# arnauqb/GradABM-JUNE

Hardware: AMD Instinct MI355X
Metric: simulation steps/sec (higher is better)
Workload: dtype f32

## Files before the change

### gradabm-june_amd/csrc/gj_tiled.h

```cpp
#pragma once
#include <hip/hip_runtime.h>
#include <stdint.h>

#include "../../include/gradjune_hip.h"
#include "gj_device.h"

namespace gj {

constexpr int kTileThreads = 1024;
constexpr int kTileWaves = kTileThreads / kWave;
constexpr int kMaxSliceAgents = 19840;
constexpr int kUnroll = 8;
#ifndef GJ_UNROLL_NARROW
#define GJ_UNROLL_NARROW 16
#endif
constexpr int kUnrollNarrow = GJ_UNROLL_NARROW;
#ifndef GJ_VENUE_UNROLL
#define GJ_VENUE_UNROLL 2
#endif
constexpr int kVenueUnroll = GJ_VENUE_UNROLL;
#ifndef GJ_VENUE_UNROLL_C
#define GJ_VENUE_UNROLL_C GJ_VENUE_UNROLL
#endif
constexpr int kVenueUnrollC = GJ_VENUE_UNROLL_C;
// ... 135 lines not shown
  b = (lane >= ((d1.z >> 24) & 0xFF)) ? d1.x : b;
  b = (lane >= (d1.w & 0xFF)) ? d1.y : b;
  return b + lane;
}
__device__ __noinline__ int chunk_slot_walk(const TSetA& T, int row, int i, int j) {
  while (i >= T.tile_sptr[row + j + 1]) ++j;
  return T.tile_jpos[row + j] + (i - T.tile_sptr[row + j]);
}

template <bool WIDE, int U>
__device__ __forceinline__ int batch_desc_load(const TSetA& T, int c_base, int n_chunks, int c0, int lane) {
  constexpr int W = WIDE ? 8 : 4;
  static_assert(U * W <= kWave, "a batch's descriptors must fit one wave-wide load");
  const int32_t* desc = reinterpret_cast<const int32_t*>(T.chunk_desc);
  const int u_l = min(lane / W, U - 1), k_l = lane % W;
  return at32(desc, (c_base + min(c0 + u_l, n_chunks - 1)) * W + k_l);
}

template <bool WIDE, int U>
__device__ __forceinline__ void batch_slots(const TSetA& T, const int word, int row, int seg0, int seg1, int c0,
                                            int lane, int (&slot)[U]) {
  constexpr int W = WIDE ? 8 : 4;
  const int k_l = lane % W;
  const bool flag = WIDE ? (k_l == 7 && (word & 0x100)) : (k_l == 2 && (word >> 16));
  const bool any_multi = __builtin_amdgcn_ballot_w64(flag) != 0ull;
#define GJ_DW(u, k) __builtin_amdgcn_readlane(word, (u) * W + (k))
  if (!any_multi) {
#pragma unroll
    for (int u = 0; u < U; ++u) {
      if (!WIDE) {
        slot[u] = chunk_slot_fast(make_int4(GJ_DW(u, 0), GJ_DW(u, 1), GJ_DW(u, 2), 0), lane);
      } else {
        slot[u] = chunk_slot_wide(make_int4(GJ_DW(u, 0), GJ_DW(u, 1), GJ_DW(u, 2), GJ_DW(u, 3)),
                                  make_int4(GJ_DW(u, 4), GJ_DW(u, 5), GJ_DW(u, 6), GJ_DW(u, 7)), lane);
      }
    }
  } else if (T.multi_slots) {
    int ms[U];
    bool mu[U];
#pragma unroll
    for (int u = 0; u < U; ++u) {
      const int w = WIDE ? GJ_DW(u, 7) : GJ_DW(u, 2);
      mu[u] = WIDE ? ((w & 0x100) != 0) : ((w >> 16) != 0);
      const int j0 = WIDE ? (int)((unsigned)w >> 9) : GJ_DW(u, 3);
      ms[u] = at32(T.multi_slots, (mu[u] ? j0 : 0) * kWave + lane);
    }
#pragma unroll
    for (int u = 0; u < U; ++u) {
      int f;
      if (!WIDE) {
        f = chunk_slot_fast(make_int4(GJ_DW(u, 0), GJ_DW(u, 1), GJ_DW(u, 2), 0), lane);
      } else {
        f = chunk_slot_wide(make_int4(GJ_DW(u, 0), GJ_DW(u, 1), GJ_DW(u, 2), GJ_DW(u, 3)),
                            make_int4(GJ_DW(u, 4), GJ_DW(u, 5), GJ_DW(u, 6), GJ_DW(u, 7)), lane);
      }
      slot[u] = mu[u] ? ms[u] : f;
    }
  } else {
#pragma unroll
    for (int u = 0; u < U; ++u) {
      const int i = min(seg0 + (c0 + u) * kWave + lane, seg1 - 1);
      if (!WIDE) {
        const int4 d = make_int4(GJ_DW(u, 0), GJ_DW(u, 1), GJ_DW(u, 2), GJ_DW(u, 3));
        slot[u] = (d.z >> 16) ? chunk_slot_slow(T, d, row, i, lane) : chunk_slot_fast(d, lane);
      } else {
        const int4 d0 = make_int4(GJ_DW(u, 0), GJ_DW(u, 1), GJ_DW(u, 2), GJ_DW(u, 3));
        const int4 d1 = make_int4(GJ_DW(u, 4), GJ_DW(u, 5), GJ_DW(u, 6), GJ_DW(u, 7));
        slot[u] = (d1.w & 0x100) ? chunk_slot_walk(T, row, i, (int)((unsigned)d1.w >> 9))
                                 : chunk_slot_wide(d0, d1, lane);
      }
    }
  }
#undef GJ_DW
}

#ifndef GJ_SCATTER_PIPELINE
#define GJ_SCATTER_PIPELINE 1
#endif
template <bool WIDE, int kU, bool NT = false>
__device__ __forceinline__ void scatter_batches(const TSetA& T, const float* lds_x, int s, int wave, int lane) {
  const int row = s * T.J;
  const int seg0 = T.tile_sptr[row], seg1 = T.tile_sptr[row + T.J];
  const int c_base = T.chunk_ptr[s];
  const int n_chunks = T.chunk_ptr[s + 1] - c_base;
  constexpr int kStride = kTileWaves * kU;
  auto stage1 = [&](int c, int& word, int (&la)[kU]) {
    const int cc = min(c, n_chunks - 1);
    word = batch_desc_load<WIDE, kU>(T, c_base, n_chunks, cc, lane);
#pragma unroll
    for (int u = 0; u < kU; ++u) la[u] = at32(T.a_la, min(seg0 + (cc + u) * kWave + lane, seg1 - 1));
  };
  auto stage2 = [&](int c, int word, const int (&la)[kU]) {
    int slot[kU];
    batch_slots<WIDE, kU>(T, word, row, seg0, seg1, c, lane, slot);
#ifdef GJ_DIAG_EXTRA_VALU
#pragma unroll
    for (int u = 0; u < kU; ++u)
#pragma unroll
      for (int r = 0; r < GJ_DIAG_EXTRA_VALU; ++r) asm volatile("v_add_u32 %0, %0, 0" : "+v"(slot[u]));
#endif
#pragma unroll
    for (int u = 0; u < kU; ++u) {
      const int i = seg0 + (c + u) * kWave + lane;
      if ((c + u < n_chunks) && (i < seg1)) {
        if (NT) put32nt(T.val, slot[u], lds_x[la[u]]); else put32(T.val, slot[u], lds_x[la[u]]);
      }
    }
  };
  int c0 = wave * kU;
  if (c0 >= n_chunks) return;
  int laA[kU], wordA;
#if GJ_SCATTER_PIPELINE
  int laB[kU], wordB;
  stage1(c0, wordA, laA);
  while (true) {
    const int c1 = c0 + kStride;
    stage1(c1, wordB, laB);
    stage2(c0, wordA, laA);
    if (c1 >= n_chunks) break;
    const int c2 = c1 + kStride;
    stage1(c2, wordA, laA);
    stage2(c1, wordB, laB);
    if (c2 >= n_chunks) break;
    c0 = c2;
  }
#else
  for (; c0 < n_chunks; c0 += kStride) {
    stage1(c0, wordA, laA);
    stage2(c0, wordA, laA);
  }
#endif
}

constexpr int kLongSegmentChunks = 384;
#ifndef GJ_NT_TILE_EDGES
#define GJ_NT_TILE_EDGES 1024
#endif
constexpr int kNtTileEdges = GJ_NT_TILE_EDGES;
template <bool WIDE>
__device__ __forceinline__ void scatter_set(const TSetA& T, const float* lds_x, int s, int wave, int lane) {
  const int n_chunks = T.chunk_ptr[s + 1] - T.chunk_ptr[s];
  if (!WIDE && kUnrollNarrow != kUnroll && n_chunks >= kLongSegmentChunks && n_chunks * kWave >= kNtTileEdges * T.J) {
    scatter_batches<WIDE, WIDE ? kUnroll : kUnrollNarrow, true>(T, lds_x, s, wave, lane);
  } else if (!WIDE && kUnrollNarrow != kUnroll && n_chunks >= kLongSegmentChunks) {
    scatter_batches<WIDE, WIDE ? kUnroll : kUnrollNarrow>(T, lds_x, s, wave, lane);
  } else {
    scatter_batches<WIDE, kUnroll>(T, lds_x, s, wave, lane);
  }
}

#ifndef GJ_UNROLL_D_NARROW
#define GJ_UNROLL_D_NARROW 8
#endif
#ifndef GJ_GATHER_PIPELINE
#define GJ_GATHER_PIPELINE 1
#endif
template <bool WIDE>
__device__ __forceinline__ void gather_set(const TSetA& T, fx_t* lds_acc, uint32_t* lds_flags, int flag_words, int s,
                                           int wave, int lane) {
  const int row = s * T.J;
  const int seg0 = T.tile_sptr[row], seg1 = T.tile_sptr[row + T.J];
  const int c_base = T.chunk_ptr[s];
  const int n_chunks = T.chunk_ptr[s + 1] - c_base;
  constexpr int kU = WIDE ? kUnroll : GJ_UNROLL_D_NARROW;
  constexpr int kStride = kTileWaves * kU;
  auto stage1 = [&](int c, int& word, int (&la)[kU]) {
    const int cc = min(c, n_chunks - 1);
    word = batch_desc_load<WIDE, kU>(T, c_base, n_chunks, cc, lane);
#pragma unroll
    for (int u = 0; u < kU; ++u) la[u] = at32(T.a_la, min(seg0 + (cc + u) * kWave + lane, seg1 - 1));
  };
  auto values = [&](int c, int word, float (&v)[kU]) {
    int slot[kU];
    batch_slots<WIDE, kU>(T, word, row, seg0, seg1, c, lane, slot);
#pragma unroll
    for (int u = 0; u < kU; ++u) {
      const int i = seg0 + (c + u) * kWave + lane;
      const bool ok = (c + u < n_chunks) && (i < seg1);
      v[u] = at32nt(T.val, ok ? slot[u] : 0);
    }
  };
  auto add = [&](int c, const int (&la)[kU], const float (&v)[kU]) {
    constexpr uint32_t kLimit = 0x48800000u;
    static_assert(kFxAgent == 32, "kLimit is the pattern of 2^(50 - kFxAgent)");
    float x[kU];
    uint32_t m = 0u;
#pragma unroll
    for (int u = 0; u < kU; ++u) {
      const int i = seg0 + (c + u) * kWave + lane;
      const bool edge = (c + u < n_chunks) && (i < seg1);
      x[u] = edge ? v[u] : 0.0f;
      m = max(m, __float_as_uint(x[u]) & 0x7FFFFFFFu);
    }
#ifdef GJ_DIAG_EXTRA_VALU
#pragma unroll
    for (int u = 0; u < kU; ++u)
#pragma unroll
      for (int r = 0; r < GJ_DIAG_EXTRA_VALU; ++r) asm volatile("v_add_f32 %0, %0, 0" : "+v"(x[u]));
#endif
    if (__builtin_expect(m <= kLimit, 1)) {
#pragma unroll
      for (int u = 0; u < kU; ++u) atomicAdd(&lds_acc[la[u]], to_fx<kFxAgent>(x[u]));
    } else {
#pragma unroll
      for (int u = 0; u < kU; ++u) {
        if ((__float_as_uint(x[u]) & 0x7FFFFFFFu) <= kLimit) {
          atomicAdd(&lds_acc[la[u]], to_fx<kFxAgent>(x[u]));
        } else {
          fx_flag(lds_flags, flag_words, la[u], x[u]);
        }
      }
    }
  };
  int c0 = wave * kU;
  if (c0 >= n_chunks) return;
  int laA[kU], wordA;
  float v[kU];
#if GJ_GATHER_PIPELINE
  int laB[kU], wordB;
  stage1(c0, wordA, laA);
  while (true) {
    const int c1 = c0 + kStride;
    values(c0, wordA, v);
    stage1(c1, wordB, laB);
    add(c0, laA, v);
    if (c1 >= n_chunks) break;
    const int c2 = c1 + kStride;
    values(c1, wordB, v);
    stage1(c2, wordA, laA);
    add(c1, laB, v);
    if (c2 >= n_chunks) break;
    c0 = c2;
  }
#else
  for (; c0 < n_chunks; c0 += kStride) {
    stage1(c0, wordA, laA);
    values(c0, wordA, v);
    add(c0, laA, v);
  }
#endif
}

template <int kU>
__device__ __forceinline__ void scatter_explicit(const TSetA& T, const float* lds_x, int s, int wave, int lane) {
  const int row = s * T.J;
  const int seg0 = T.tile_sptr[row], seg1 = T.tile_sptr[row + T.J];
  const int n_chunks = T.chunk_ptr[s + 1] - T.chunk_ptr[s];
  const int32_t* slots = reinterpret_cast<const int32_t*>(T.chunk_desc);
  for (int c0 = wave * kU; c0 < n_chunks; c0 += kTileWaves * kU) {
    int la[kU], sl[kU];
#pragma unroll
    for (int u = 0; u < kU; ++u) {
      const int i = min(seg0 + (c0 + u) * kWave + lane, seg1 - 1);
      la[u] = at32(T.a_la, i);
      sl[u] = at32(slots, i);
    }
#pragma unroll
    for (int u = 0; u < kU; ++u) {
      const int i = seg0 + (c0 + u) * kWave + lane;
      if ((c0 + u < n_chunks) && (i < seg1)) put32(T.val, sl[u], lds_x[la[u]]);
    }
  }
}

template <int kU>
__device__ __forceinline__ void gather_explicit(const TSetA& T, fx_t* lds_acc, uint32_t* lds_flags, int flag_words, int s,
                                                int wave, int lane) {
  const int row = s * T.J;
  const int seg0 = T.tile_sptr[row], seg1 = T.tile_sptr[row + T.J];
  const int n_chunks = T.chunk_ptr[s + 1] - T.chunk_ptr[s];
  const int32_t* slots = reinterpret_cast<const int32_t*>(T.chunk_desc);
  constexpr uint32_t kLimit = 0x48800000u;
  for (int c0 = wave * kU; c0 < n_chunks; c0 += kTileWaves * kU) {
    int la[kU], sl[kU];
#pragma unroll
    for (int u = 0; u < kU; ++u) {
      const int i = min(seg0 + (c0 + u) * kWave + lane, seg1 - 1);
      la[u] = at32(T.a_la, i);
      sl[u] = at32(slots, i);
    }
    float x[kU];
#pragma unroll
    for (int u = 0; u < kU; ++u) x[u] = at32(T.val, sl[u]);
    uint32_t m = 0u;
#pragma unroll
    for (int u = 0; u < kU; ++u) {
      const int i = seg0 + (c0 + u) * kWave + lane;
      x[u] = ((c0 + u < n_chunks) && (i < seg1)) ? x[u] : 0.0f;
      m = max(m, __float_as_uint(x[u]) & 0x7FFFFFFFu);
    }
    if (__builtin_expect(m <= kLimit, 1)) {
#pragma unroll
      for (int u = 0; u < kU; ++u) atomicAdd(&lds_acc[la[u]], to_fx<kFxAgent>(x[u]));
    } else {
#pragma unroll
      for (int u = 0; u < kU; ++u) {
        if ((__float_as_uint(x[u]) & 0x7FFFFFFFu) <= kLimit) {
          atomicAdd(&lds_acc[la[u]], to_fx<kFxAgent>(x[u]));
        } else {
          fx_flag(lds_flags, flag_words, la[u], x[u]);
        }
      }
    }
  }
}

#ifndef GJ_SCATTER_WAVES_PER_SIMD
#define GJ_SCATTER_WAVES_PER_SIMD 4
#endif
__global__ __launch_bounds__(kTileThreads, GJ_SCATTER_WAVES_PER_SIMD) void k_tile_scatter(const TileAArgs A) {
  extern __shared__ __align__(16) float lds_x[];
  const int tid = threadIdx.x;
  const int wave = __builtin_amdgcn_readfirstlane(tid / kWave), lane = tid % kWave;
  const int s = blockIdx.x;
  const int64_t base = (int64_t)s * A.slice_agents;
  const int n_local = (int)min((int64_t)A.slice_agents, A.n_agents - base);
  const bool two_sources = A.qtrans != A.trans;
  for (int pass = 0; pass < 2; ++pass) {
    if (pass == 1 && !two_sources) break;
    bool any = false;
    for (int t = 0; t < A.n_sets; ++t)
      if (A.sets[t].active && !A.sets[t].presum && (!two_sources || A.sets[t].raw == pass)) any = true;
    if (!any) continue;
    if (pass == 1) __syncthreads();
    load_slice(lds_x, pass == 0 ? A.qtrans : A.trans, base, n_local, tid);
    __syncthreads();
    for (int t = 0; t < A.n_sets; ++t) {
      const TSetA& T = A.sets[t];
      if (!T.active || T.presum || (two_sources && T.raw != pass)) continue;
      if (T.wide == 2) {
        scatter_explicit<kUnroll>(T, lds_x, s, wave, lane);
      } else if (T.wide) {
        scatter_set<true>(T, lds_x, s, wave, lane);
      } else {
        scatter_set<false>(T, lds_x, s, wave, lane);
      }
    }
  }
}

struct TSetB {
  const int32_t* blk_v0;
  const int32_t* blk_e0;
  const uint16_t* e_lv;
  const uint8_t* e_cls;
  float* val;
  const float* v_pc;
  float* cum;
  int32_t stride;
  int32_t nk;
  float beta[GJ_MAX_NETS_PER_SET];
  int32_t table[GJ_MAX_NETS_PER_SET];
  int32_t age75[GJ_MAX_NETS_PER_SET];
  int32_t leisure;
  int32_t direct;
  uint32_t term_limit;
  int32_t _pad_b;
  const uint16_t* pv_blk;
  const int32_t* blk_r0;
  const float* x;
  int64_t n_x;
};

struct TileBArgs {
  TSetB sets[GJ_MAX_SETS];
  const int32_t* work;
  const float* tables;
  int32_t day_type;
  int32_t mode;
  int32_t transpose;
  int32_t _pad;
};

__device__ __noinline__ void venue_group_slow(fx_t* sums, uint32_t* vflags, int words, uint32_t limit, int base_k, int l0,
                                              int l1, int l2, int l3, int l4, int l5, int l6, int l7, float x0, float x1,
                                              float x2, float x3, float x4, float x5, float x6, float x7) {
  const int lv[8] = {l0, l1, l2, l3, l4, l5, l6, l7};
  const float x[8] = {x0, x1, x2, x3, x4, x5, x6, x7};
#pragma unroll
  for (int q = 0; q < 8; ++q) {
    if (lv[q] == 0xFFFF) continue;
    if ((__float_as_uint(x[q]) & 0x7FFFFFFFu) <= limit) {
      atomicAdd(&sums[base_k + lv[q]], to_fx<kFxVenue>(x[q]));
    } else {
      fx_flag(vflags, words, base_k + lv[q], x[q]);
    }
  }
}

struct Slots8 {
  uint32_t w[4];
  __device__ __forceinline__ int lv(int q) const { return (w[q >> 1] >> ((q & 1) * 16)) & 0xFFFF; }
};

#ifdef GJ_DIAG_STAMPS
constexpr int kDiagVenueSlots = 8192;
__device__ unsigned long long gj_diag_venue[3 * kDiagVenueSlots];
struct VenueStamp {
  unsigned long long t0;
  __device__ VenueStamp() : t0(__builtin_amdgcn_s_memrealtime()) {}
  __device__ ~VenueStamp() {
    if (threadIdx.x == 0 && blockIdx.x < kDiagVenueSlots) {
      gj_diag_venue[3 * blockIdx.x] = t0;
      gj_diag_venue[3 * blockIdx.x + 1] = __builtin_amdgcn_s_memrealtime();
      gj_diag_venue[3 * blockIdx.x + 2] = __builtin_amdgcn_s_getreg((31 << 11) | 20) & 0xF;
    }
  }
};
#endif

#ifndef GJ_VENUE_WAVES_PER_SIMD
#define GJ_VENUE_WAVES_PER_SIMD 4
#endif
__global__ __launch_bounds__(kTileThreads, GJ_VENUE_WAVES_PER_SIMD) void k_tile_venues(const TileBArgs B) {
  extern __shared__ __align__(16) float lds_s[];
#ifdef GJ_DIAG_STAMPS
  VenueStamp gj_stamp;
#endif
  const int tid = threadIdx.x;
  const int set = B.work[2 * blockIdx.x], j = B.work[2 * blockIdx.x + 1];
  const TSetB& T = B.sets[set];
  const int nk = T.nk;
  if (nk == 0) return;
  const int v0 = T.blk_v0[j], nv = T.blk_v0[j + 1] - v0;
  const int g0 = T.blk_e0[j] >> 3, g1 = T.blk_e0[j + 1] >> 3;
  fx_t* sums = reinterpret_cast<fx_t*>(lds_s);
  float* cumf = lds_s;
  float* tabs = lds_s + 2 * ((size_t)nk * nv + 64);
  uint32_t* vflags = reinterpret_cast<uint32_t*>(tabs + (T.leisure ? 2 * nk * 200 : 0));
  const int vwords = (nk * nv + 64 + 31) / 32;
  if (T.leisure) {
    for (int i = tid; i < nk * 200; i += kTileThreads) {
      const int k = i / 200, c = i % 200;
      const float l = B.tables[(int64_t)T.table[k] * GJ_TABLE_SIZE + B.day_type * 200 + c];
      const float lw = T.age75[k] ? l * (((c % 100) > 75) ? 1.0f : 0.0f) : l;
      tabs[i] = B.transpose ? lw : l;
      tabs[nk * 200 + i] = B.transpose ? l : lw;
    }
  }
  const uint4* lv8 = reinterpret_cast<const uint4*>(T.e_lv);
  const uint2* cls8 = reinterpret_cast<const uint2*>(T.e_cls);
  float4* val4 = reinterpret_cast<float4*>(T.val);
  if (B.mode != 2) {
    for (int i = tid; i < nk * nv + 64; i += kTileThreads) sums[i] = 0;
    for (int i = tid; i < 2 * vwords; i += kTileThreads) vflags[i] = 0u;
    __syncthreads();
    const int dummy = nk * nv + (tid & 63);
#if defined(GJ_DIAG_FLOAT_RUNS)
    auto run_sums = [&](const int (&lv)[8], const float (&x)[8], int base_k) {
      float s8 = x[0];
#pragma unroll
      for (int q = 0; q < 8; ++q) {
        const bool last = (q == 7) || (lv[q + (q < 7)] != lv[q]);
        const bool take = last && lv[q] != 0xFFFF;
        fx_add<kFxVenue>(sums, vflags, vwords, take ? base_k + lv[q] : dummy, take ? s8 : 0.0f);
// ... 544 lines not shown
        for (int c = 0; c < K; ++c) x[j][c] = tab[idx[j][c] * stride];
    } else {
#pragma unroll
      for (int j = 0; j < 4; ++j)
#pragma unroll
        for (int c = 0; c < K; ++c) x[j][c] = 0.0f;
#pragma unroll
      for (int k = 0; k < GJ_MAX_NETS_PER_SET; ++k) {
        if (k >= nk) break;
        float w[4];
#pragma unroll
        for (int j = 0; j < 4; ++j) w[j] = wtab[k * 200 + ((b.cls[u] >> (8 * j)) & 0xFF)];
#pragma unroll
        for (int j = 0; j < 4; ++j)
#pragma unroll
          for (int c = 0; c < K; ++c) x[j][c] += w[j] * tab[idx[j][c] * stride + k];
      }
    }
#pragma unroll
    for (int j = 0; j < 4; ++j) {
      float sj = 0.0f;
#pragma unroll
      for (int c = 0; c < K; ++c) sj += ok[j][c] ? x[j][c] : 0.0f;
      acc[u][j] += sj;
    }
  }
}

__device__ __forceinline__ void direct_stage(const TileDArgs& D, const TDirect& T, float* wtab, float* tab, int v0,
                                             int nv, int tid) {
  if (T.leisure && v0 == 0) {
    for (int i = tid; i < T.nk * 200; i += kTileThreads) {
      const int k = i / 200, c = i % 200;
      const float l = D.tables[(int64_t)T.table[k] * GJ_TABLE_SIZE + D.day_type * 200 + c];
      const float lw = T.age75[k] ? l * (((c % 100) > 75) ? 1.0f : 0.0f) : l;
      wtab[i] = D.transpose ? l : lw;
    }
  }
#ifndef GJ_DIAG_NO_DIRECT_TABLE
  const float* src = T.cum + (int64_t)v0 * T.stride;
  const int n = nv * T.stride;
  const int lane = tid % kWave, wave = __builtin_amdgcn_readfirstlane(tid / kWave);
#if GJ_DMA_WIDE
  const bool aligned = ((reinterpret_cast<uintptr_t>(src) | reinterpret_cast<uintptr_t>(tab)) & 15u) == 0;
  const int n_wide = aligned ? (n / (4 * kWave)) * (4 * kWave) : 0;
  for (int p = wave; (p + 1) * 4 * kWave <= n_wide; p += kTileWaves)
    __builtin_amdgcn_global_load_lds(src + p * 4 * kWave + 4 * lane, tab + p * 4 * kWave, 16, 0, 0);
  for (int p = wave; n_wide + p * kWave < n; p += kTileWaves)
    __builtin_amdgcn_global_load_lds(src + min(n_wide + p * kWave + lane, n - 1), tab + n_wide + p * kWave, 4, 0, 0);
#else
  for (int p = wave; p * kWave < n; p += kTileWaves)
    __builtin_amdgcn_global_load_lds(src + min(p * kWave + lane, n - 1), tab + p * kWave, 4, 0, 0);
#endif
#endif
}

__device__ __forceinline__ void publish_staged() {
  asm volatile("s_waitcnt vmcnt(0)" ::: "memory");
  __syncthreads();
}

__device__ __forceinline__ bool direct_next(const TileDArgs& D, int& t, int& v0, int& plane) {
  const TDirect& T = D.direct[t];
  if (plane + 1 < T.planes) {
    ++plane;
    return true;
  }
  plane = 0;
  if (!T.win_lo && v0 + T.group_venues < T.V) {
    v0 += T.group_venues;
    return true;
  }
  v0 = 0;
  ++t;
  return t < D.n_direct;
}

__device__ __forceinline__ void direct_sets(const TileDArgs& D, float (&acc)[kQuadsPerLane][4], uint32_t qmask,
                                            float* lds, int64_t base, int n_local, int tid, DirectBatch& cur,
                                            uint64_t diag_t0 = 0) {
  auto wtab_of = [&](int t) { return lds + (t & 1) * kClassWeightFloats; };
  auto tab_of = [&](const TDirect& T) {
    return lds + 2 * kClassWeightFloats + (T.region ? D.table_floats + kWave : 0);
  };
  auto group_nv = [&](const TDirect& T, int v0) { return T.win_lo ? T.win_n[blockIdx.x] : min(T.group_venues, T.V - v0); };
  auto group_lo = [&](const TDirect& T, int v0) { return T.win_lo ? T.win_lo[blockIdx.x] : v0; };
  int t = 0, v0 = 0, plane = 0;
  __syncthreads();
  direct_stage(D, D.direct[0], wtab_of(0), tab_of(D.direct[0]), group_lo(D.direct[0], 0), group_nv(D.direct[0], 0), tid);
  bool more = true;
  while (more) {
    const TDirect& T = D.direct[t];
    const int nv = group_nv(T, v0);
    if (plane == 0) publish_staged();
#ifdef GJ_DIAG_STAMPS
    if (threadIdx.x == 0 && D.trans_susc && t < 4)
      D.trans_susc[(int64_t)blockIdx.x * D.slice_agents + 8 + 2 * t] = (float)(__builtin_amdgcn_s_memtime() - diag_t0);
#endif
    int tn = t, vn = v0, pn = plane;
    more = direct_next(D, tn, vn, pn);
    const bool new_group = more && pn == 0;
    const bool overlap = new_group && D.direct[tn].region != T.region;
    if (overlap)
      direct_stage(D, D.direct[tn], wtab_of(tn), tab_of(D.direct[tn]), group_lo(D.direct[tn], vn), group_nv(D.direct[tn], vn), tid);
    DirectBatch nxt;
    if (more) direct_load(D, D.direct[tn], base, n_local, tid, pn, nxt);
#ifndef GJ_DIAG_NO_DIRECT_ADD
    direct_add(D, T, acc, qmask, wtab_of(t), tab_of(T), v0, nv, n_local, tid, cur);
#else
    if (cur.w[0][0] == 0x12345678u && cur.cls[0] == 77u) acc[0][0] = 1.0f;
#endif
#ifdef GJ_DIAG_STAMPS
    if (threadIdx.x == 0 && D.trans_susc && t < 4)
      D.trans_susc[(int64_t)blockIdx.x * D.slice_agents + 9 + 2 * t] = (float)(__builtin_amdgcn_s_memtime() - diag_t0);
#endif
    if (new_group && !overlap) {
      __syncthreads();
      direct_stage(D, D.direct[tn], wtab_of(tn), tab_of(D.direct[tn]), group_lo(D.direct[tn], vn), group_nv(D.direct[tn], vn), tid);
    }
    if (more) cur = nxt;
    t = tn;
    v0 = vn;
    plane = pn;
  }
}

__device__ __forceinline__ void load_quad(const float* p, int64_t a0, int n_ok, bool vec, float (&v)[4]) {
  if (vec && n_ok >= 4) {
    const float4 x = *reinterpret_cast<const float4*>(p + a0);
    v[0] = x.x;
    v[1] = x.y;
    v[2] = x.z;
    v[3] = x.w;
  } else {
#pragma unroll
    for (int j = 0; j < 4; ++j) v[j] = (j < n_ok) ? p[a0 + j] : 0.0f;
  }
}
template <bool NT = false>
__device__ __forceinline__ void store_quad(float* p, int64_t a0, int n_ok, bool vec, const float (&v)[4]) {
  if (vec && n_ok >= 4) {
    if (NT) {
      store_nt(reinterpret_cast<float4*>(p + a0), make_float4(v[0], v[1], v[2], v[3]));
    } else {
      *reinterpret_cast<float4*>(p + a0) = make_float4(v[0], v[1], v[2], v[3]);
    }
  } else {
#pragma unroll
    for (int j = 0; j < 4; ++j)
      if (j < n_ok) p[a0 + j] = v[j];
  }
}

#ifdef GJ_DIAG_STAMPS
#define GJ_STAMP(k)                                                                                         \
  do {                                                                                                      \
    if (threadIdx.x == 0 && D.trans_susc)                                                                    \
      D.trans_susc[(int64_t)blockIdx.x * D.slice_agents + (k)] = (float)(__builtin_amdgcn_s_memtime() - gj_t0); \
  } while (0)
#else
#define GJ_STAMP(k) do { } while (0)
#endif

__global__ __launch_bounds__(kTileThreads) void k_tile_agents(const TileDArgs D) {
  extern __shared__ __align__(16) fx_t lds_acc[];
#ifdef GJ_DIAG_STAMPS
  const uint64_t gj_t0 = __builtin_amdgcn_s_memtime();
#endif
  const int tid = threadIdx.x;
  const int wave = __builtin_amdgcn_readfirstlane(tid / kWave), lane = tid % kWave;
  const int s = blockIdx.x;
  const int64_t base = (int64_t)s * D.slice_agents;
  const int n_local = (int)min((int64_t)D.slice_agents, D.n_agents - base);
  uint32_t* lds_flags = reinterpret_cast<uint32_t*>(lds_acc + D.slice_agents);
  const int fwords = D.slice_agents / 32;
  for (int i = tid; i < n_local; i += kTileThreads) lds_acc[i] = 0;
  for (int i = tid; i < 2 * fwords; i += kTileThreads) lds_flags[i] = 0u;
  DirectBatch first;
  if (D.n_direct > 0) direct_load(D, D.direct[0], base, n_local, tid, 0, first);
  __syncthreads();
  for (int pass = 0; pass < 2; ++pass) {
    for (int t = 0; t < D.n_sets; ++t) {
      const TSetA& T = D.sets[t];
      if (!T.active || T.direct || T.raw != pass) continue;
      if (T.wide == 2) {
        gather_explicit<kUnroll>(T, lds_acc, lds_flags, fwords, s, wave, lane);
      } else if (T.wide) {
        gather_set<true>(T, lds_acc, lds_flags, fwords, s, wave, lane);
      } else {
        gather_set<false>(T, lds_acc, lds_flags, fwords, s, wave, lane);
      }
    }
    __syncthreads();
    if (pass == 0 && D.has_q) {
      constexpr int kStageBatch = 10;
      for (int i0 = tid; i0 < n_local; i0 += kStageBatch * kTileThreads) {
        float stg[kStageBatch];
#pragma unroll
        for (int u = 0; u < kStageBatch; ++u) stg[u] = D.stage[base + min(i0 + u * kTileThreads, n_local - 1)];
#pragma unroll
        for (int u = 0; u < kStageBatch; ++u) {
          const int i = i0 + u * kTileThreads;
          if (i < n_local && !(stg[u] < D.q_thr)) {
            lds_acc[i] = 0;
            const uint32_t bit = 1u << (i & 31);
            const bool pos = lds_flags[i >> 5] & bit, neg = lds_flags[fwords + (i >> 5)] & bit;
            if (pos != neg) {
              atomicAnd(&lds_flags[i >> 5], ~bit);
              atomicAnd(&lds_flags[fwords + (i >> 5)], ~bit);
            }
          }
        }
      }
      __syncthreads();
    }
  }
  GJ_STAMP(1);
  constexpr int kQ = kQuadsPerLane;
  float acc[kQ][4];
#pragma unroll
  for (int m = 0; m < kQ; ++m) {
    const int i0 = 4 * (tid + m * kTileThreads);
    const int iq = min(i0, D.slice_agents - 4);
    const uint32_t pos = (lds_flags[iq >> 5] >> (iq & 31)) & 0xFu, neg = (lds_flags[fwords + (iq >> 5)] >> (iq & 31)) & 0xFu;
    fx_t raw[4];
#pragma unroll
    for (int j = 0; j < 4; ++j) raw[j] = lds_acc[iq + j];
#pragma unroll
    for (int j = 0; j < 4; ++j) {
      const float v = from_fx<kFxAgent>(raw[j]);
      acc[m][j] = (i0 < n_local) ? (((pos | neg) >> j) & 1u ? fx_special((pos >> j) & 1u, (neg >> j) & 1u, v) : v) : 0.0f;
    }
  }
  if (D.n_direct > 0) {
    uint32_t qmask = 0u;
    if (D.has_q) {
      float stg[kQ][4];
#pragma unroll
      for (int m = 0; m < kQ; ++m) {
        const int i0 = 4 * (tid + m * kTileThreads);
#pragma unroll
        for (int j = 0; j < 4; ++j) stg[m][j] = (i0 + j < n_local) ? D.stage[base + i0 + j] : -INFINITY;
      }
#pragma unroll
      for (int m = 0; m < kQ; ++m)
#pragma unroll
        for (int j = 0; j < 4; ++j) qmask |= (stg[m][j] < D.q_thr) ? 0u : (1u << (4 * m + j));
    }
    GJ_STAMP(2);
#ifndef GJ_DIAG_NO_DIRECT_SETS
#ifdef GJ_DIAG_STAMPS
    direct_sets(D, acc, qmask, reinterpret_cast<float*>(lds_acc), base, n_local, tid, first, gj_t0);
#else
    direct_sets(D, acc, qmask, reinterpret_cast<float*>(lds_acc), base, n_local, tid, first);
#endif
#endif
    GJ_STAMP(3);
  }
  const bool vec = D.io_vec4 != 0;
  if (D.agent_sums) {
#pragma unroll
    for (int m = 0; m < kQ; ++m) {
      const int i0 = 4 * (tid + m * kTileThreads);
      if (i0 < n_local) store_quad<true>(D.agent_sums, base + i0, n_local - i0, vec, acc[m]);
    }
  }
  if (D.acc_scratch) {
#pragma unroll
    for (int m = 0; m < kQ; ++m) {
      const int i0 = 4 * (tid + m * kTileThreads);
      if (i0 < n_local) store_quad(D.acc_scratch, base + i0, n_local - i0, vec, acc[m]);
    }
    return;
  }
  const float now = D.clock ? D.clock->now : D.now;
  const uint64_t step = D.clock ? D.clock->step : D.step;
  const bool own_noise = D.sample && !D.exp_noise;
  const int mis = (int)((D.agent_offset + base) & 3);
  float4* ts4 = reinterpret_cast<float4*>(lds_acc);
  {
    float sq[kQ][4];
#pragma unroll
    for (int m = 0; m < kQ; ++m) {
      int i0 = 4 * (tid + m * kTileThreads);
      asm volatile("" : "+v"(i0));
#pragma unroll
      for (int j = 0; j < 4; ++j) sq[m][j] = 0.0f;
      if (i0 < n_local) load_quad(D.susceptibility, base + i0, n_local - i0, vec, sq[m]);
    }
    __syncthreads();
#pragma unroll
    for (int m = 0; m < kQ; ++m) {
      const int q = tid + m * kTileThreads;
      if (4 * q < n_local)
        ts4[q] = make_float4(sq[m][0] * acc[m][0], sq[m][1] * acc[m][1], sq[m][2] * acc[m][2], sq[m][3] * acc[m][3]);
    }
  }
  GJ_STAMP(4);
  uint32_t infected = 0u;
  int m_run = 0;
  for (int q = tid; 4 * q < n_local; q += kTileThreads, ++m_run) {
    const int i0 = 4 * q;
    const float4 tq = ts4[q];
    const float ts[4] = {tq.x, tq.y, tq.z, tq.w};
    const int64_t a0 = base + i0;
    const int n_ok = n_local - i0;
    float p[4];
#pragma unroll
    for (int j = 0; j < 4; ++j) p[j] = not_infected_prob(ts[j], D.dt);
#ifndef GJ_DIAG_STAMPS
    if (D.trans_susc) store_quad<true>(D.trans_susc, a0, n_ok, vec, ts);
#endif
    if (D.not_infected_probs) store_quad<true>(D.not_infected_probs, a0, n_ok, vec, p);
    if (!D.sample) continue;
    float nw[4], th[4] = {0.0f, 0.0f, 0.0f, 0.0f};
    if (own_noise) {
      const uint64_t g0 = (uint64_t)(D.agent_offset + a0);
      uint32_t r0[4], r1[4] = {0u, 0u, 0u, 0u};
      philox4x32_10(g0 >> 2, step, D.seed, r0);
      if (mis) philox4x32_10((g0 >> 2) + 1, step, D.seed, r1);
#pragma unroll
      for (int j = 0; j < 4; ++j) {
        const int w = mis + j;
        th[j] = u01(w == 0 ? r0[0] : w == 1 ? r0[1] : w == 2 ? r0[2] : w == 3 ? r0[3] : w == 4 ? r1[0] : w == 5 ? r1[1] : r1[2]);
      }
    }
#pragma unroll
    for (int j = 0; j < 4; ++j) {
      if (own_noise) {
        nw[j] = own_new_infected(p[j], th[j]);
      } else {
        float e0 = 1.0f, e1 = 1.0f;
        if (j < n_ok) {
          e0 = D.exp_noise[a0 + j];
          e1 = D.exp_noise[D.n_agents + a0 + j];
        }
        nw[j] = gumbel_new_infected(p[j], e0, e1);
      }
      if (j < n_ok && nw[j] != 0.0f) infected |= 1u << (4 * m_run + j);
    }
    if (D.new_infected) store_quad<true>(D.new_infected, a0, n_ok, vec, nw);
#pragma unroll
    for (int j = 0; j < 4; ++j) {
      if (j < n_ok && nw[j] != 0.0f && nw[j] != 1.0f) {
        infected &= ~(1u << (4 * m_run + j));
        const int64_t a = a0 + j;
        float sc = D.susceptibility[a], inf = D.is_infected[a], t_inf = D.infection_time[a];
        infect(nw[j], now, sc, inf, t_inf);
        D.susceptibility[a] = sc;
        D.is_infected[a] = inf;
        D.infection_time[a] = t_inf;
      }
    }
  }
  GJ_STAMP(6);
#ifndef GJ_TAIL_BATCHED
  if (__builtin_amdgcn_ballot_w64(infected != 0u) != 0ull) {
    uint32_t todo = infected;
    while (todo) {
      const int k = __builtin_ctz(todo);
      todo &= todo - 1u;
      const int64_t a = base + 4 * (tid + (k >> 2) * kTileThreads) + (k & 3);
      float sc = D.susceptibility[a], inf = D.is_infected[a], tinf = D.infection_time[a];
      infect(1.0f, now, sc, inf, tinf);
      D.susceptibility[a] = sc;
      D.is_infected[a] = inf;
      D.infection_time[a] = tinf;
    }
  }
// ... 34 lines not shown
```

Measured before the change: 1947.

## Pipeline gather prefetch across transmission sets and unify explicit gather path

Replaces the per-set gather functions with one gather_run that, when a set's last chunk is consumed, issues the first descriptor and slot loads of the next active set. This hides the load latency at set boundaries. The explicit (wide==2) gather now uses the same software-pipelined loop instead of a serial loop. The direct_load prefetch moves after the gather passes and gains an extra barrier, and a pass-1 barrier is dropped. Register pressure rises because buffers are sized to the larger unroll and the next-set header is kept live.

```diff
diff --git a/gradabm-june_amd/csrc/gj_tiled.h b/gradabm-june_amd/csrc/gj_tiled.h
--- a/gradabm-june_amd/csrc/gj_tiled.h
+++ b/gradabm-june_amd/csrc/gj_tiled.h
@@ -311,35 +311,86 @@
 #ifndef GJ_UNROLL_D_NARROW
 #define GJ_UNROLL_D_NARROW 8
 #endif
-#ifndef GJ_GATHER_PIPELINE
-#define GJ_GATHER_PIPELINE 1
-#endif
-template <bool WIDE>
-__device__ __forceinline__ void gather_set(const TSetA& T, fx_t* lds_acc, uint32_t* lds_flags, int flag_words, int s,
-                                           int wave, int lane) {
-  const int row = s * T.J;
-  const int seg0 = T.tile_sptr[row], seg1 = T.tile_sptr[row + T.J];
-  const int c_base = T.chunk_ptr[s];
-  const int n_chunks = T.chunk_ptr[s + 1] - c_base;
-  constexpr int kU = WIDE ? kUnroll : GJ_UNROLL_D_NARROW;
+#ifndef GJ_GATHER_ACROSS_SETS
+#define GJ_GATHER_ACROSS_SETS 1
+#endif
+constexpr int kGatherNarrow = 0, kGatherWide = 1, kGatherExplicit = 2;
+constexpr int kGatherU = GJ_UNROLL_D_NARROW > kUnroll ? GJ_UNROLL_D_NARROW : kUnroll;
+
+struct GatherHdr {
+  int t, pass;
+  int row, seg0, seg1, c_base, n_chunks;
+};
+
+#ifdef GJ_DIAG_STAMPS
+struct GatherDiag {
+  float* out;
+  uint64_t t0;
+  int k;
+};
+#define GJ_GATHER_STAMP(g, which)                                                                               \
+  do {                                                                                                          \
+    if (threadIdx.x == 0 && (g).out && (g).k < 8)                                                               \
+      (g).out[16 + 2 * (g).k + (which)] = (float)(__builtin_amdgcn_s_memtime() - (g).t0);                       \
+  } while (0)
+#else
+struct GatherDiag {};
+#define GJ_GATHER_STAMP(g, which) do { } while (0)
+#endif
+
+template <int FORM>
+__device__ __forceinline__ void gather_first(const TSetA& T, const GatherHdr& h, int c, int lane, int& word,
+                                             int (&p)[kGatherU]) {
+  constexpr int kU = FORM == kGatherNarrow ? GJ_UNROLL_D_NARROW : kUnroll;
+  const int cc = min(c, h.n_chunks - 1);
+  if (FORM == kGatherExplicit) {
+    const int32_t* slots = reinterpret_cast<const int32_t*>(T.chunk_desc);
+    word = 0;
+#pragma unroll
+    for (int u = 0; u < kU; ++u) p[u] = at32(slots, min(h.seg0 + (cc + u) * kWave + lane, h.seg1 - 1));
+  } else {
+    word = batch_desc_load<FORM == kGatherWide, kU>(T, h.c_base, h.n_chunks, cc, lane);
+#pragma unroll
+    for (int u = 0; u < kU; ++u) p[u] = at32(T.a_la, min(h.seg0 + (cc + u) * kWave + lane, h.seg1 - 1));
+  }
+}
+__device__ __forceinline__ void gather_first_of_set(const TSetA& T, const GatherHdr& h, int wave, int lane, int& word,
+                                                    int (&p)[kGatherU]) {
+  if (T.wide == kGatherExplicit) {
+    if (wave * kUnroll < h.n_chunks) gather_first<kGatherExplicit>(T, h, wave * kUnroll, lane, word, p);
+  } else if (T.wide) {
+    if (wave * kUnroll < h.n_chunks) gather_first<kGatherWide>(T, h, wave * kUnroll, lane, word, p);
+  } else {
+    if (wave * GJ_UNROLL_D_NARROW < h.n_chunks) gather_first<kGatherNarrow>(T, h, wave * GJ_UNROLL_D_NARROW, lane, word, p);
+  }
+}
+
+template <int FORM, typename Next>
+__device__ __forceinline__ void gather_run(const TSetA& T, const GatherHdr& h, fx_t* lds_acc, uint32_t* lds_flags,
+                                           int flag_words, int wave, int lane, int& wordA, int (&pA)[kGatherU],
+                                           Next&& issue_next, GatherDiag diag) {
+  constexpr bool WIDE = FORM == kGatherWide;
+  constexpr int kU = FORM == kGatherNarrow ? GJ_UNROLL_D_NARROW : kUnroll;
   constexpr int kStride = kTileWaves * kU;
-  auto stage1 = [&](int c, int& word, int (&la)[kU]) {
-    const int cc = min(c, n_chunks - 1);
-    word = batch_desc_load<WIDE, kU>(T, c_base, n_chunks, cc, lane);
-#pragma unroll
-    for (int u = 0; u < kU; ++u) la[u] = at32(T.a_la, min(seg0 + (cc + u) * kWave + lane, seg1 - 1));
+  const int row = h.row, seg0 = h.seg0, seg1 = h.seg1, n_chunks = h.n_chunks;
+  auto values = [&](int c, int word, const int (&p)[kGatherU], int (&la)[kGatherU], float (&v)[kGatherU]) {
+    if (FORM == kGatherExplicit) {
+#pragma unroll
+      for (int u = 0; u < kU; ++u) v[u] = at32(T.val, p[u]);
+#pragma unroll
+      for (int u = 0; u < kU; ++u) la[u] = at32(T.a_la, min(seg0 + (c + u) * kWave + lane, seg1 - 1));
+    } else {
+      int slot[kU];
+      batch_slots<WIDE, kU>(T, word, row, seg0, seg1, c, lane, slot);
+#pragma unroll
+      for (int u = 0; u < kU; ++u) {
+        const int i = seg0 + (c + u) * kWave + lane;
+        const bool ok = (c + u < n_chunks) && (i < seg1);
+        v[u] = at32nt(T.val, ok ? slot[u] : 0);
+      }
+    }
   };
-  auto values = [&](int c, int word, float (&v)[kU]) {
-    int slot[kU];
-    batch_slots<WIDE, kU>(T, word, row, seg0, seg1, c, lane, slot);
-#pragma unroll
-    for (int u = 0; u < kU; ++u) {
-      const int i = seg0 + (c + u) * kWave + lane;
-      const bool ok = (c + u < n_chunks) && (i < seg1);
-      v[u] = at32nt(T.val, ok ? slot[u] : 0);
-    }
-  };
-  auto add = [&](int c, const int (&la)[kU], const float (&v)[kU]) {
+  auto add = [&](int c, const int (&la)[kGatherU], const float (&v)[kGatherU]) {
     constexpr uint32_t kLimit = 0x48800000u;
     static_assert(kFxAgent == 32, "kLimit is the pattern of 2^(50 - kFxAgent)");
     float x[kU];
@@ -372,32 +423,35 @@
     }
   };
   int c0 = wave * kU;
-  if (c0 >= n_chunks) return;
-  int laA[kU], wordA;
-  float v[kU];
-#if GJ_GATHER_PIPELINE
-  int laB[kU], wordB;
-  stage1(c0, wordA, laA);
+  if (c0 >= n_chunks) {
+    issue_next(wordA, pA);
+    return;
+  }
+  int pB[kGatherU] = {}, wordB = 0;
+  int la[kGatherU];
+  float v[kGatherU];
+  bool first = true;
   while (true) {
     const int c1 = c0 + kStride;
-    values(c0, wordA, v);
-    stage1(c1, wordB, laB);
-    add(c0, laA, v);
-    if (c1 >= n_chunks) break;
+    values(c0, wordA, pA, la, v);
+    if (c1 < n_chunks) gather_first<FORM>(T, h, c1, lane, wordB, pB); else issue_next(wordB, pB);
+    add(c0, FORM == kGatherExplicit ? la : pA, v);
+    if (first) GJ_GATHER_STAMP(diag, 0);
+    first = false;
+    if (c1 >= n_chunks) {
+      wordA = wordB;
+#pragma unroll
+      for (int u = 0; u < kGatherU; ++u) pA[u] = pB[u];
+      break;
+    }
     const int c2 = c1 + kStride;
-    values(c1, wordB, v);
-    stage1(c2, wordA, laA);
-    add(c1, laB, v);
+    values(c1, wordB, pB, la, v);
+    if (c2 < n_chunks) gather_first<FORM>(T, h, c2, lane, wordA, pA); else issue_next(wordA, pA);
+    add(c1, FORM == kGatherExplicit ? la : pB, v);
     if (c2 >= n_chunks) break;
     c0 = c2;
   }
-#else
-  for (; c0 < n_chunks; c0 += kStride) {
-    stage1(c0, wordA, laA);
-    values(c0, wordA, v);
-    add(c0, laA, v);
-  }
-#endif
+  GJ_GATHER_STAMP(diag, 1);
 }
 
 template <int kU>
@@ -418,48 +472,6 @@
     for (int u = 0; u < kU; ++u) {
       const int i = seg0 + (c0 + u) * kWave + lane;
       if ((c0 + u < n_chunks) && (i < seg1)) put32(T.val, sl[u], lds_x[la[u]]);
-    }
-  }
-}
-
-template <int kU>
-__device__ __forceinline__ void gather_explicit(const TSetA& T, fx_t* lds_acc, uint32_t* lds_flags, int flag_words, int s,
-                                                int wave, int lane) {
-  const int row = s * T.J;
-  const int seg0 = T.tile_sptr[row], seg1 = T.tile_sptr[row + T.J];
-  const int n_chunks = T.chunk_ptr[s + 1] - T.chunk_ptr[s];
-  const int32_t* slots = reinterpret_cast<const int32_t*>(T.chunk_desc);
-  constexpr uint32_t kLimit = 0x48800000u;
-  for (int c0 = wave * kU; c0 < n_chunks; c0 += kTileWaves * kU) {
-    int la[kU], sl[kU];
-#pragma unroll
-    for (int u = 0; u < kU; ++u) {
-      const int i = min(seg0 + (c0 + u) * kWave + lane, seg1 - 1);
-      la[u] = at32(T.a_la, i);
-      sl[u] = at32(slots, i);
-    }
-    float x[kU];
-#pragma unroll
-    for (int u = 0; u < kU; ++u) x[u] = at32(T.val, sl[u]);
-    uint32_t m = 0u;
-#pragma unroll
-    for (int u = 0; u < kU; ++u) {
-      const int i = seg0 + (c0 + u) * kWave + lane;
-      x[u] = ((c0 + u < n_chunks) && (i < seg1)) ? x[u] : 0.0f;
-      m = max(m, __float_as_uint(x[u]) & 0x7FFFFFFFu);
-    }
-    if (__builtin_expect(m <= kLimit, 1)) {
-#pragma unroll
-      for (int u = 0; u < kU; ++u) atomicAdd(&lds_acc[la[u]], to_fx<kFxAgent>(x[u]));
-    } else {
-#pragma unroll
-      for (int u = 0; u < kU; ++u) {
-        if ((__float_as_uint(x[u]) & 0x7FFFFFFFu) <= kLimit) {
-          atomicAdd(&lds_acc[la[u]], to_fx<kFxAgent>(x[u]));
-        } else {
-          fx_flag(lds_flags, flag_words, la[u], x[u]);
-        }
-      }
     }
   }
 }
@@ -1310,6 +1322,24 @@
   }
 }
 
+__device__ __forceinline__ bool gather_next(const TileDArgs& D, int s, int pass, int t, GatherHdr& h) {
+  for (; pass < 2; ++pass, t = 0) {
+    for (; t < D.n_sets; ++t) {
+      const TSetA& T = D.sets[t];
+      if (!T.active || T.direct || T.raw != pass) continue;
+      h.t = t;
+      h.pass = pass;
+      h.row = s * T.J;
+      h.seg0 = T.tile_sptr[h.row];
+      h.seg1 = T.tile_sptr[h.row + T.J];
+      h.c_base = T.chunk_ptr[s];
+      h.n_chunks = T.chunk_ptr[s + 1] - h.c_base;
+      return true;
+    }
+  }
+  return false;
+}
+
 #ifdef GJ_DIAG_STAMPS
 #define GJ_STAMP(k)                                                                                         \
   do {                                                                                                      \
@@ -1325,34 +1355,64 @@
 #ifdef GJ_DIAG_STAMPS
   const uint64_t gj_t0 = __builtin_amdgcn_s_memtime();
 #endif
-  const int tid = threadIdx.x;
-  const int wave = __builtin_amdgcn_readfirstlane(tid / kWave), lane = tid % kWave;
+  const int tid0 = threadIdx.x;
+  const int wave = __builtin_amdgcn_readfirstlane(tid0 / kWave), lane = tid0 % kWave;
   const int s = blockIdx.x;
   const int64_t base = (int64_t)s * D.slice_agents;
   const int n_local = (int)min((int64_t)D.slice_agents, D.n_agents - base);
   uint32_t* lds_flags = reinterpret_cast<uint32_t*>(lds_acc + D.slice_agents);
   const int fwords = D.slice_agents / 32;
-  for (int i = tid; i < n_local; i += kTileThreads) lds_acc[i] = 0;
-  for (int i = tid; i < 2 * fwords; i += kTileThreads) lds_flags[i] = 0u;
+  for (int i = tid0; i < n_local; i += kTileThreads) lds_acc[i] = 0;
+  for (int i = tid0; i < 2 * fwords; i += kTileThreads) lds_flags[i] = 0u;
+  auto tid_again = [&]() {
+    int l = lane;
+    asm volatile("" : "+v"(l));
+    return wave * kWave + l;
+  };
   DirectBatch first;
-  if (D.n_direct > 0) direct_load(D, D.direct[0], base, n_local, tid, 0, first);
+  GatherHdr cur, nxt;
+  int g_word = 0, g_p[kGatherU] = {};
+  bool have = gather_next(D, s, 0, 0, cur);
+#if GJ_GATHER_ACROSS_SETS
+  if (have) gather_first_of_set(D.sets[cur.t], cur, wave, lane, g_word, g_p);
+#endif
+  GatherDiag diag;
+#ifdef GJ_DIAG_STAMPS
+  diag.out = D.trans_susc ? D.trans_susc + (int64_t)blockIdx.x * D.slice_agents : nullptr;
+  diag.t0 = gj_t0;
+  diag.k = 0;
+#endif
   __syncthreads();
   for (int pass = 0; pass < 2; ++pass) {
-    for (int t = 0; t < D.n_sets; ++t) {
-      const TSetA& T = D.sets[t];
-      if (!T.active || T.direct || T.raw != pass) continue;
-      if (T.wide == 2) {
-        gather_explicit<kUnroll>(T, lds_acc, lds_flags, fwords, s, wave, lane);
+    while (have && cur.pass == pass) {
+      const TSetA& T = D.sets[cur.t];
+      const bool have_next = gather_next(D, s, cur.pass, cur.t + 1, nxt);
+#if GJ_GATHER_ACROSS_SETS
+      auto issue_next = [&](int& word, int (&p)[kGatherU]) {
+        if (have_next) gather_first_of_set(D.sets[nxt.t], nxt, wave, lane, word, p);
+      };
+#else
+      auto issue_next = [](int&, int (&)[kGatherU]) {};
+      gather_first_of_set(T, cur, wave, lane, g_word, g_p);
+#endif
+      if (T.wide == kGatherExplicit) {
+        gather_run<kGatherExplicit>(T, cur, lds_acc, lds_flags, fwords, wave, lane, g_word, g_p, issue_next, diag);
       } else if (T.wide) {
-        gather_set<true>(T, lds_acc, lds_flags, fwords, s, wave, lane);
+        gather_run<kGatherWide>(T, cur, lds_acc, lds_flags, fwords, wave, lane, g_word, g_p, issue_next, diag);
       } else {
-        gather_set<false>(T, lds_acc, lds_flags, fwords, s, wave, lane);
-      }
-    }
+        gather_run<kGatherNarrow>(T, cur, lds_acc, lds_flags, fwords, wave, lane, g_word, g_p, issue_next, diag);
+      }
+#ifdef GJ_DIAG_STAMPS
+      ++diag.k;
+#endif
+      cur = nxt;
+      have = have_next;
+    }
+    if (pass == 1) break;
     __syncthreads();
-    if (pass == 0 && D.has_q) {
+    if (D.has_q) {
       constexpr int kStageBatch = 10;
-      for (int i0 = tid; i0 < n_local; i0 += kStageBatch * kTileThreads) {
+      for (int i0 = tid_again(); i0 < n_local; i0 += kStageBatch * kTileThreads) {
         float stg[kStageBatch];
 #pragma unroll
         for (int u = 0; u < kStageBatch; ++u) stg[u] = D.stage[base + min(i0 + u * kTileThreads, n_local - 1)];
@@ -1373,6 +1433,9 @@
       __syncthreads();
     }
   }
+  const int tid = tid_again();
+  if (D.n_direct > 0) direct_load(D, D.direct[0], base, n_local, tid, 0, first);
+  __syncthreads();
   GJ_STAMP(1);
   constexpr int kQ = kQuadsPerLane;
   float acc[kQ][4];
```

New measurement: 1937, median of 2. Within noise of the previous version (-0.5%).
